# jhardenberg/smmregrid

Measured on NVIDIA B200. Metric: regridded source points/sec, 0.1deg->1deg remapcon, higher is better.
Workload: dtype f64

## Files before the change

### include/smmregrid_b200.h

```cpp
#ifndef SMMREGRID_B200_H
#define SMMREGRID_B200_H

#include <stdint.h>

#ifdef __cplusplus
extern "C" {
#endif

#define SMM_OK 0
#define SMM_ERR_INVALID 1
#define SMM_ERR_RANGE 2
#define SMM_ERR_CUDA 3
#define SMM_ERR_ALLOC 4
#define SMM_ERR_DTYPE 5

#define SMM_F32 0
#define SMM_F64 1
#define SMM_I16 2

#define SMM_KERNEL_STAGED 1
#define SMM_KERNEL_GATHER 2
#define SMM_KERNEL_COMPACT 3

#define SMM_SUM_AUTO 0
// ... 100 lines not shown

typedef struct smm_host_plan smm_host_plan;
int smm_host_plan_build(int64_t n_src, int64_t n_dst, int64_t nnz,
                        const int32_t *src_address, const int32_t *dst_address,
                        const double *remap_matrix, int32_t num_wgts, int32_t index_base,
                        const smm_create_opts *opts, smm_host_plan **out);
int smm_host_plan_info(const smm_host_plan *p, smm_info *out, int64_t *n_segs_out);
int smm_host_plan_copy(const smm_host_plan *p, int32_t *rowptr, int32_t *col, double *val,
                       int32_t *tiles, uint32_t *segs, double *wplan, uint16_t *iplan);
int smm_host_plan_rowmap(const smm_host_plan *p, int32_t *rowmap);
int smm_host_plan_gather_rows(const smm_host_plan *p, int32_t *rows);
int smm_host_plan_rowslot(const smm_host_plan *p, int32_t *rowslot);
int smm_host_plan_compact(const smm_host_plan *p, int64_t *n_touched_out, int64_t *n_blocks_out,
                          int32_t *tcols, int32_t *blk_ptr, int32_t *rcol);
void smm_host_plan_free(smm_host_plan *p);

int smm_copy_ceiling(int32_t device, void *host, int64_t bytes, int32_t direction, int32_t reps,
                     double *seconds_out);

int64_t smm_launch_count(void);

const char *smm_last_error(void);
const char *smm_version(void);

#ifdef __cplusplus
}
#endif
#endif
```

### smmregrid_b200/_lib.py

```python
from __future__ import annotations

import ctypes
import os

from . import _build

SMM_OK, SMM_ERR_INVALID, SMM_ERR_RANGE, SMM_ERR_CUDA, SMM_ERR_ALLOC, SMM_ERR_DTYPE = range(6)
SMM_F32, SMM_F64, SMM_I16 = 0, 1, 2
SMM_KERNEL_STAGED, SMM_KERNEL_GATHER, SMM_KERNEL_COMPACT = 1, 2, 3
KERNEL_NAMES = {SMM_KERNEL_STAGED: "staged", SMM_KERNEL_GATHER: "gather"}
KERNEL_CODES = {None: 0, "auto": 0, "staged": SMM_KERNEL_STAGED, "gather": SMM_KERNEL_GATHER,
                "compact": SMM_KERNEL_COMPACT}
SMM_SUM_AUTO, SMM_SUM_FAST, SMM_SUM_REFERENCE = 0, 1, 2
SUMMATION_CODES = {None: SMM_SUM_AUTO, "auto": SMM_SUM_AUTO, "fast": SMM_SUM_FAST, "reference": SMM_SUM_REFERENCE}
SUMMATION_NAMES = {SMM_SUM_FAST: "fast", SMM_SUM_REFERENCE: "reference"}

i32, i64, f64 = ctypes.c_int32, ctypes.c_int64, ctypes.c_double
vp = ctypes.c_void_p
P = ctypes.POINTER


class SmmInfo(ctypes.Structure):
    _fields_ = [
        ("n_src", i64), ("n_dst", i64), ("nnz", i64),
# ... 50 lines not shown
    "smm_set_dst_mask": (ctypes.c_int, [vp, i32, vp, vp]),
    "smm_apply": (ctypes.c_int, [vp, i32, vp, i32, i64, i64, vp, i32, i64, i32, f64, P(SmmApplyOpts), vp]),
    "smm_apply_levels": (ctypes.c_int, [vp, i32, vp, vp, i32, i64, i64, i64, vp, i32, i64, i64, vp, f64,
                                        P(SmmApplyOpts), vp]),
    "smm_apply_host": (ctypes.c_int, [vp, i32, vp, i32, i64, i64, vp, i32, i64, i32, f64, P(SmmApplyOpts), i64]),
    "smm_apply_levels_host": (ctypes.c_int, [vp, i32, vp, vp, i32, i64, vp, i32, vp, f64, P(SmmApplyOpts), i64]),
    "smm_nan_variation": (ctypes.c_int, [vp, i32, i64, i64, i64, P(i64), vp]),
    "smm_host_plan_build": (ctypes.c_int, [i64, i64, i64, vp, vp, vp, i32, i32, P(SmmCreateOpts), P(vp)]),
    "smm_host_plan_info": (ctypes.c_int, [vp, P(SmmInfo), P(i64)]),
    "smm_host_plan_copy": (ctypes.c_int, [vp, vp, vp, vp, vp, vp, vp, vp]),
    "smm_host_plan_rowmap": (ctypes.c_int, [vp, vp]),
    "smm_host_plan_rowslot": (ctypes.c_int, [vp, vp]),
    "smm_host_plan_gather_rows": (ctypes.c_int, [vp, vp]),
    "smm_host_plan_compact": (ctypes.c_int, [vp, P(i64), P(i64), vp, vp, vp]),
    "smm_host_plan_free": (None, [vp]),
    "smm_copy_ceiling": (ctypes.c_int, [i32, vp, i64, i32, i32, P(f64)]),
    "smm_launch_count": (i64, []),
    "smm_last_error": (ctypes.c_char_p, []),
    "smm_version": (ctypes.c_char_p, []),
}

_lib = None


class SmmError(RuntimeError):
    pass


def lib_path() -> str:
    return os.environ.get("SMM_LIB_PATH") or _build.LIB_PATH
# ... 28 lines not shown
```

### smmregrid_b200/csrc/smm_api.cu

```cuda
#include <cuda_runtime.h>

#include <algorithm>
#include <atomic>
#include <chrono>
#include <cmath>
#include <cstdio>
#include <cstdlib>
#include <cstring>
#include <mutex>
#include <string>
#include <thread>
#include <vector>

#include <sched.h>
#if defined(__x86_64__) || defined(_M_X64)
#include <emmintrin.h>
#endif

#include "../../include/smmregrid_b200.h"
#include "smm_internal.h"
#include "smm_aux_kernels.cuh"
#include "smm_plan.h"

using namespace smm;
// ... 331 lines not shown
    return e ? std::atoi(e) : dflt;
}

#define SMM_DTYPE_DISPATCH(FN, ...)                                                                           \
    ((x_dtype == SMM_I16)                                                                                     \
         ? ((opt.dec_dtype == SMM_F32)                                                                        \
                ? (y_dtype == SMM_F32 ? FN<I16F32, float>(__VA_ARGS__) : FN<I16F32, double>(__VA_ARGS__))     \
                : (y_dtype == SMM_F32 ? FN<I16F64, float>(__VA_ARGS__) : FN<I16F64, double>(__VA_ARGS__)))    \
     : (x_dtype == SMM_F32 && y_dtype == SMM_F32) ? FN<float, float>(__VA_ARGS__)                             \
     : (x_dtype == SMM_F32 && y_dtype == SMM_F64) ? FN<float, double>(__VA_ARGS__)                            \
     : (x_dtype == SMM_F64 && y_dtype == SMM_F32) ? FN<double, float>(__VA_ARGS__)                            \
                                                  : FN<double, double>(__VA_ARGS__))

size_t x_elem_bytes(int32_t x_dtype) { return x_dtype == SMM_I16 ? 2 : x_dtype == SMM_F32 ? 4 : 8; }

int64_t pick_chunks(int64_t B, int64_t blocks_total, int64_t slots, double bytes_per_row, double prologue_us,
                    int64_t multiple, int64_t &chunk)
{
    static const int k_min_rows = std::max(1, env_int("SMM_MIN_ROWS_PER_ITEM", 8));
    static const int k_waves = env_int("SMM_WAVES", 0);
    const double t_us = static_cast<double>(B) * bytes_per_row / 6.5e6;
    double waves = k_waves > 0 ? k_waves : std::sqrt(t_us / (2.0 * prologue_us));
    waves = std::min(32.0, std::max(1.0, waves));
    const double items = waves * static_cast<double>(slots);
    int64_t nchunks = static_cast<int64_t>(items / static_cast<double>(std::max<int64_t>(blocks_total, 1)) + 0.5);
    const int64_t max_chunks = std::max<int64_t>(1, B / k_min_rows);
    nchunks = std::max<int64_t>(1, std::min<int64_t>({nchunks, max_chunks, 65535}));
    chunk = (B + nchunks - 1) / nchunks;
    chunk = (chunk + multiple - 1) / multiple * multiple;
    return (B + chunk - 1) / chunk;
}

constexpr int kCompactUnavailable = -1;

struct ApplyOpts {
    int kernel = 0;
    double renorm_min_valid = -1.0;
// ... 103 lines not shown
        if (!ok && opt.kernel == SMM_KERNEL_STAGED)
            return fail(SMM_ERR_INVALID, "staged kernel forced but unavailable for level " +
                                             std::to_string(s.level) + ": " +
                                             (L.staged ? std::string("slab alignment / footprint size")
                                                       : L.why_not_staged));
        (ok ? staged : gather).push_back(s);
        if (ok && L.n_gather_rows > 0) gather_lists.push_back(s);
    }

    ApplyArgs a{};
    a.B = B; a.x_bstride = xbs; a.y_bstride = ybs; a.remap_area_min = area_min;
    a.renorm_min_valid = opt.renorm_min_valid;
    a.dec = opt.dec;
    static const uint32_t k_debug_flags = static_cast<uint32_t>(env_int("SMM_DEBUG_STREAM_ONLY", 0)) & 3u;
    static const int k_max_stages = std::max(2, env_int("SMM_MAX_STAGES", kMaxStages));
    a.debug_flags = k_debug_flags;

    auto fill_job = [&](const JobSpec &s, LevelJob &j) {
        const LevelDev &L = h->levels[s.level];
        j.tiles = L.tiles; j.segs = L.segs; j.wplan = L.wplan; j.iplan = L.iplan; j.rowmap = L.rowmap;
        j.rowptr = L.rowptr; j.col = L.col; j.val = L.val;
        j.imask = L.imask; j.frac = L.frac;
        j.x = s.x; j.y = s.y; j.masked = s.masked; j.nrows = 0;
    };

    const size_t staged_groups = (staged.size() + kMaxJobs - 1) / kMaxJobs;
    const size_t staged_per = staged_groups ? (staged.size() + staged_groups - 1) / staged_groups : 1;
    for (size_t g0 = 0; g0 < staged.size();) {
        size_t g1 = g0;
        JobBatch jb{};
// ... 24 lines not shown
        {
            const size_t budget = (nct == 256 ? half : h->smem_optin) - std::min(stage_off, half);
            nb_rows = static_cast<int>(std::min<size_t>(nb_rows, std::max<size_t>(1, budget / (4 * row_bytes))));
        }
        nb_rows = static_cast<int>(std::max<int64_t>(1, std::min<int64_t>({nb_rows, 8, B})));
        if (ordl) {
            nb_rows = (B >= 2 && stage_off + 4 * row_bytes <= h->smem_optin) ? 2 : 1;
            while (nb_rows >= 2 && nb_rows + 2 <= 8 && nb_rows + 2 <= B &&
                   stage_off + 3 * static_cast<size_t>(nb_rows + 2) * row_bytes <= h->smem_optin)
                nb_rows += 2;
        }
        const size_t stage_bytes = row_bytes * nb_rows;
        int64_t chunk = 0;
        const double row_bytes_hbm = static_cast<double>(g1 - g0) *
                                     (static_cast<double>(a.n_src) * sx + static_cast<double>(a.n_dst) * (y_dtype == SMM_F32 ? 4 : 8));
        const int ctas_per_sm = (!ordl && nct == 256) ? 2 : 1;
        const int64_t nchunks = pick_chunks(B, tiles_total, static_cast<int64_t>(h->sm_count) * ctas_per_sm,
                                            row_bytes_hbm, ordl ? 6.0 : (nct == 256 ? 2.5 : 4.0), nb_rows, chunk);
        a.chunk = chunk; a.nchunks = static_cast<int32_t>(nchunks);
        size_t S = (!ordl && nct == 256 && half > stage_off) ? (half - stage_off) / stage_bytes : 0;
        if (S < 3) S = (h->smem_optin - stage_off) / stage_bytes;
        S = std::min<size_t>(S, kMaxStages);
        S = std::min<size_t>(S, static_cast<size_t>(k_max_stages));
        if (S < 2) return fail(SMM_ERR_INVALID, "internal: staged footprint does not fit");
        a.nstages = static_cast<int32_t>(S);
        a.stage_bytes = static_cast<uint32_t>(stage_bytes);
        a.row_bytes = static_cast<uint32_t>(row_bytes);
        a.rows_per_stage = nb_rows;
        a.stage_off = static_cast<uint32_t>(stage_off);
        const size_t smem = stage_off + S * stage_bytes;
        int64_t max_tiles = 0;
        jb.njobs = static_cast<int32_t>(g1 - g0);
        for (size_t g = g0; g < g1; ++g) {
            LevelJob &j = jb.jobs[g - g0];
            fill_job(staged[g], j);
            j.nblocks = h->levels[staged[g].level].ntiles;
            j.item0 = 0;
            max_tiles = std::max<int64_t>(max_tiles, j.nblocks);
        }
        g0 = g1;
        if (max_tiles == 0) continue;
        const dim3 grid(static_cast<unsigned>(max_tiles), static_cast<unsigned>(nchunks), static_cast<unsigned>(jb.njobs));
        static const int k_ord_tpr = env_int("SMM_ORD_TPR", 0);
        const int tpr = (ordl && nb_rows >= 2 && (k_ord_tpr == 2 || (k_ord_tpr == 0 && nct <= 128))) ? 2 : 1;
        const int rc = ordl ? SMM_DTYPE_DISPATCH(launch_ordered_t, h->device, nct, tpr, grid, smem, st, jb, a)
                            : SMM_DTYPE_DISPATCH(launch_staged_t, h->device, lpr, kpl, nct, packed, ord, grid, smem, st, jb, a);
        if (rc) return rc;
    }

    {
        std::vector<JobSpec> plain;
        for (const JobSpec &sp : gather) {
            const LevelDev &L = h->levels[sp.level];
            const double gather_cost = static_cast<double>(L.nnz) * 120.0;
            const double compact_cost = 1.2 * (static_cast<double>(L.n_src) + static_cast<double>(L.touched) +
                                               static_cast<double>(L.nnz)) * static_cast<double>(sx);
            bool use = L.rcol && opt.renorm_min_valid < 0.0 && opt.kernel != SMM_KERNEL_GATHER;
// ... 582 lines not shown
    smm_host_plan *p = new (std::nothrow) smm_host_plan();
    if (!p) return fail(SMM_ERR_ALLOC, "host allocation failed");
    std::vector<HostCsr> csrs;
    std::vector<HostPlan> plans;
    bool ref_order = false;
    const int64_t ll = nnz;
    const int rc = build_host_operator(1, &ll, nnz, n_src, n_dst, src_address, dst_address, remap_matrix, num_wgts,
                                       index_base, opts, 148, csrs, plans, ref_order, p->cache_hit);
    if (rc) { delete p; return rc; }
    p->csr = std::move(csrs[0]);
    p->plan = std::move(plans[0]);
    *out = p;
    return SMM_OK;
}

int smm_host_plan_info(const smm_host_plan *p, smm_info *out, int64_t *n_segs_out)
{
    if (!p || !out) return fail(SMM_ERR_INVALID, "null argument");
    std::memset(out, 0, sizeof(*out));
    out->n_src = p->csr.n_src; out->n_dst = p->csr.n_dst;
    out->nnz = static_cast<int64_t>(p->csr.col.size());
    out->n_levels = 1;
    out->kernel = p->plan.ok ? SMM_KERNEL_STAGED : SMM_KERNEL_GATHER;
    out->lanes_per_row = p->plan.lpr; out->links_per_lane = p->plan.kpl;
    out->rows_per_tile = p->plan.rows_per_tile;
    out->n_tiles = p->plan.ok ? static_cast<int32_t>(p->plan.tiles.size()) : 0;
    out->max_row_nnz = p->csr.max_row_nnz;
    out->max_tile_segments = p->plan.max_tile_segments;
    out->consumer_threads = p->plan.nct;
    out->rows_reordered = (p->plan.ok && p->plan.reordered) ? 1 : 0;
// ... 107 lines not shown
```

### smmregrid_b200/csrc/smm_common.h

```cpp
#pragma once
#include <cstdint>

namespace smm {

constexpr int kMaxConsumerThreads = 512;
constexpr int kMaxStages = 12;
constexpr int kSegAlign = 8;
constexpr int kSegGap = 32;
constexpr int kSmemHeader = 256;
constexpr int kMaxJobs = 128;
constexpr int kGatherThreads = 256;
constexpr int kGatherBT = 4;

#ifndef SMM_COMPACT_BC
#define SMM_COMPACT_BC 64
#endif
#ifndef SMM_COMPACT_W
#define SMM_COMPACT_W 256
#endif
constexpr int kCompactBC = SMM_COMPACT_BC;
constexpr int kCompactW = SMM_COMPACT_W;

struct Seg {
    uint32_t src;
// ... 32 lines not shown

struct JobBatch {
    LevelJob jobs[kMaxJobs];
    int32_t njobs;
    int32_t pad;
};

struct Decode {
    double scale, offset;
    float scale_f, offset_f;
    int32_t fill[4];
    uint32_t sign_xor;
    float bias_f;
};

struct ApplyArgs {
    int64_t B;
    int64_t x_bstride;
    int64_t y_bstride;
    int64_t n_src, n_dst;
    int64_t chunk;
    int32_t nchunks;
    int32_t nstages;
    uint32_t stage_bytes;
    uint32_t row_bytes;
    int32_t rows_per_stage;
    uint32_t stage_off;
    double remap_area_min;
    double renorm_min_valid;
    uint32_t debug_flags;
    int32_t ord_k;
    uint32_t wimg_off, oimg_off;
    Decode dec;
};

}
```

### smmregrid_b200/csrc/smm_kernels.cuh

```cuda
#pragma once
#include <cuda_runtime.h>
#include <math_constants.h>
#include <cuda/std/type_traits>

#include "smm_common.h"

namespace smm {


__device__ __forceinline__ uint32_t smem_u32(const void *p)
{
    return static_cast<uint32_t>(__cvta_generic_to_shared(p));
}
__device__ __forceinline__ void mbar_init(uint32_t bar, uint32_t count)
{
    asm volatile("mbarrier.init.shared::cta.b64 [%0], %1;" ::"r"(bar), "r"(count) : "memory");
}
__device__ __forceinline__ void mbar_fence_init()
{
    asm volatile("fence.mbarrier_init.release.cluster;" ::: "memory");
}
__device__ __forceinline__ void mbar_arrive(uint32_t bar)
{
    asm volatile("mbarrier.arrive.shared::cta.b64 _, [%0];" ::"r"(bar) : "memory");
// ... 166 lines not shown
#endif
}

__device__ __forceinline__ const LevelJob &find_job(const JobBatch &jb, int item, int &j)
{
    int lo = 0, hi = jb.njobs - 1;
#pragma unroll 1
    while (lo < hi) {
        const int mid = (lo + hi + 1) >> 1;
        if (item >= jb.jobs[mid].item0) lo = mid; else hi = mid - 1;
    }
    j = lo;
    return jb.jobs[j];
}


template <typename TX> __device__ __forceinline__ TX lds(uint32_t addr);
template <> __device__ __forceinline__ float lds<float>(uint32_t addr)
{
    float v;
    asm volatile("ld.shared.f32 %0, [%1];" : "=f"(v) : "r"(addr));
    return v;
}
template <> __device__ __forceinline__ double lds<double>(uint32_t addr)
{
    double v;
    asm volatile("ld.shared.f64 %0, [%1];" : "=d"(v) : "r"(addr));
    return v;
}
template <> __device__ __forceinline__ uint16_t lds<uint16_t>(uint32_t addr)
// ... 158 lines not shown
#ifndef SMM_PRODUCERS_512
#define SMM_PRODUCERS_512 4
#endif
__host__ __device__ constexpr int producer_warps(int nct) { return nct == 512 ? SMM_PRODUCERS_512 : 4; }
constexpr int kProducerRegs = 40;
#ifndef SMM_CONSUMER_REGS_512
#define SMM_CONSUMER_REGS_512 104
#endif
__host__ __device__ constexpr int consumer_regs(int nct) { return nct == 512 ? SMM_CONSUMER_REGS_512 : 96; }

struct SegB { uint32_t dst, len; uint64_t src; };

template <typename TX>
__device__ __forceinline__ void produce_stages(const LevelJob &job, const ApplyArgs &a, const TileDesc &td,
                                               const SegB *ssegs, uint32_t full_addr, uint32_t empty_addr,
                                               uint32_t stages_addr, int p, int nwarps, int lane, int64_t b0, int64_t b1)
{
    const int per_stage = td.nseg * a.rows_per_stage;
    const int active = per_stage >= 3 * nwarps ? nwarps : (per_stage + 2) / 3 > 0 ? (per_stage + 2) / 3 : 1;
    if (p >= active) return;
    const uint64_t policy = l2_evict_first_policy();
    const char *xbase = static_cast<const char *>(job.x);
    const uint32_t tile_bytes = static_cast<uint32_t>(td.elems) * sizeof(xs_t<TX>);
    const int NB = a.rows_per_stage;
    const int S = a.nstages;
    const int64_t xrow_stride = a.x_bstride * static_cast<int64_t>(sizeof(xs_t<TX>));
    int s = 0;
    uint32_t ph = 0;
    for (int64_t g = b0; g < b1; g += NB) {
        const int nb = (g + NB <= b1) ? NB : static_cast<int>(b1 - g);
        mbar_wait(empty_addr + 8 * s, ph ^ 1u);
        const uint32_t fb = full_addr + 8 * s;
        if (p == 0 && lane == 0) mbar_arrive_expect_tx(fb, tile_bytes * static_cast<uint32_t>(nb));
        const char *xg = xbase + g * xrow_stride;
        const uint32_t sbase = stages_addr + static_cast<uint32_t>(s) * a.stage_bytes;
        const int ncopies = nb * td.nseg;
        for (int i = p + active * lane; i < ncopies; i += 32 * active) {
            const int n = i / td.nseg;
            const SegB e = ssegs[i - n * td.nseg];
            tma_bulk_g2s(sbase + static_cast<uint32_t>(n) * a.row_bytes + e.dst, xg + n * xrow_stride + e.src, e.len,
                         fb, policy);
        }
        if (++s == S) { s = 0; ph ^= 1u; }
    }
}

template <typename TX, typename TY, int LPR, int KPL, int NCT, bool PACKED = false, bool ORD = false>
__global__ void __launch_bounds__(NCT + 32 * producer_warps(NCT), NCT == 256 ? 2 : 1)
staged_kernel(const __grid_constant__ JobBatch jb, const __grid_constant__ ApplyArgs a)
{
    constexpr int kProducerWarps = producer_warps(NCT);
    constexpr int kThreads = NCT + 32 * kProducerWarps;
    constexpr int kConsumerWarps = NCT / 32;
    extern __shared__ __align__(128) unsigned char smem[];
    const int tid = threadIdx.x;
    const int warp = tid >> 5;
    const int lane = tid & 31;

    const LevelJob &job = jb.jobs[blockIdx.z];
    const int tile = blockIdx.x;
    const int chunk = blockIdx.y;
    if (tile >= job.nblocks) return;
    const int64_t b0 = static_cast<int64_t>(chunk) * a.chunk;
    const int64_t b1 = (b0 + a.chunk < a.B) ? b0 + a.chunk : a.B;
    const TileDesc td = job.tiles[tile];

    SegB *ssegs = reinterpret_cast<SegB *>(smem + kSmemHeader);
    const uint32_t smem_addr = pin_reg(smem_u32(smem));
    const uint32_t full_addr = smem_addr, empty_addr = smem_addr + 8 * kMaxStages;
    const uint32_t stages_addr = smem_u32(smem) + a.stage_off;
    const int S = a.nstages;

    for (int i = tid; i < td.nseg; i += kThreads) {
        const Seg sg = job.segs[td.seg0 + i];
        ssegs[i] = SegB{sg.dst * static_cast<uint32_t>(sizeof(xs_t<TX>)), sg.len * static_cast<uint32_t>(sizeof(xs_t<TX>)),
                        static_cast<uint64_t>(sg.src) * sizeof(xs_t<TX>)};
    }
    if (tid == 0) {
        for (int s = 0; s < S; ++s) {
            mbar_init(full_addr + 8 * s, 1);
            mbar_init(empty_addr + 8 * s, kConsumerWarps);
        }
        mbar_fence_init();
    }
    __syncthreads();

    if (warp >= kConsumerWarps) {
        asm volatile("setmaxnreg.dec.sync.aligned.u32 %0;" ::"n"(kProducerRegs));
        produce_stages<TX>(job, a, td, ssegs, full_addr, empty_addr, stages_addr, warp - kConsumerWarps, kProducerWarps,
                           lane, b0, b1);
    } else {
        asm volatile("setmaxnreg.inc.sync.aligned.u32 %0;" ::"n"(consumer_regs(NCT)));
        const int r_in = tid / LPR;
        const int l_in = tid % LPR;
        const bool valid = r_in < td.nrows;
        const int row = (!PACKED && job.rowmap && valid) ? job.rowmap[td.row0 + r_in] : td.row0 + r_in;

        double w[KPL];
        uint32_t off[KPL];
        {
            const size_t base = static_cast<size_t>(tile) * KPL * NCT + tid;
#pragma unroll
            for (int k = 0; k < KPL; ++k) {
                w[k] = __ldg(job.wplan + base + static_cast<size_t>(k) * NCT);
                off[k] = stages_addr + static_cast<uint32_t>(__ldg(job.iplan + base + static_cast<size_t>(k) * NCT)) *
                                           static_cast<uint32_t>(sizeof(xs_t<TX>));
            }
        }
        if constexpr (PACKED) {
            static_assert(LPR == 1 && KPL == 16, "packed rows: 4 sub-rows of 4 links per thread");
            int rs[4];
            uint32_t flags = 0;
#pragma unroll
            for (int u = 0; u < 4; ++u) {
                rs[u] = __ldg(job.rowmap + (static_cast<size_t>(tile) * 4 + u) * NCT + tid);
                if (rs[u] == -2) flags |= 1u << u;
                if (rs[u] >= 0) {
                    bool dead = false;
                    if (job.masked && job.imask[rs[u]] == 0) dead = true;
                    if (a.remap_area_min > 0.0 && job.frac[rs[u]] < a.remap_area_min) dead = true;
                    if (dead) flags |= 16u << u;
                }
            }
            uint32_t dm[4];
#pragma unroll
            for (int u = 0; u < 4; ++u) {
                dm[u] = (flags & (16u << u)) ? 0x7ff80000u : 0u;
                asm volatile("" : "+r"(dm[u]));
            }
            TY *yb = static_cast<TY *>(job.y) + b0 * a.y_bstride;
            const xs_t<TX> *xp = static_cast<const xs_t<TX> *>(job.x) + b0 * a.x_bstride;
            const bool stream_only = (a.debug_flags & 1u) != 0;
            const int NB = a.rows_per_stage;
            bool prefer_fill = false;
            uint32_t n_done = 0;
            int s = 0;
            uint32_t ph = 0;
            for (int64_t g = b0; g < b1; g += NB) {
                const int nb = (g + NB <= b1) ? NB : static_cast<int>(b1 - g);
                mbar_wait(full_addr + 8 * s, ph);
                uint32_t sb = static_cast<uint32_t>(s) * a.stage_bytes;
#pragma unroll 1
                for (int n = 0; n < nb; ++n, sb += a.row_bytes, yb += a.y_bstride, xp += a.x_bstride) {
                    double s4[4] = {0.0, 0.0, 0.0, 0.0};
                    if (!stream_only) {
                        const bool probe = !prefer_fill || (n_done & 15u) == 0;
                        ++n_done;
                        if (probe) {
                            if constexpr (ORD) lane_chain4<TX, false>(sb, off, w, flags, s4, a.dec);
                            else lane_sum4<TX, false>(sb, off, w, s4, a.dec);
                            prefer_fill = __any_sync(0xffffffffu, not_finite((s4[0] + s4[1]) + (s4[2] + s4[3])));
                        }
                        if (prefer_fill) {
                            if constexpr (ORD) lane_chain4<TX, true>(sb, off, w, flags, s4, a.dec);
                            else lane_sum4<TX, true>(sb, off, w, s4, a.dec);
                        }
                    }
                    if (n == nb - 1) {
                        __syncwarp();
                        if (lane == 0) mbar_arrive(empty_addr + 8 * s);
                    }
                    double acc[4];
                    acc[3] = s4[3];
                    if constexpr (ORD) {
                        acc[2] = (flags & 8u) ? acc[3] : s4[2];
                        acc[1] = (flags & 4u) ? acc[2] : s4[1];
                        acc[0] = (flags & 2u) ? acc[1] : s4[0];
                    } else {
                        acc[2] = s4[2] + ((flags & 8u) ? acc[3] : 0.0);
                        acc[1] = s4[1] + ((flags & 4u) ? acc[2] : 0.0);
                        acc[0] = s4[0] + ((flags & 2u) ? acc[1] : 0.0);
                    }
                    const int hi_max = max(max(__double2hiint(acc[0]), __double2hiint(acc[1])),
                                           max(__double2hiint(acc[2]), __double2hiint(acc[3])));
                    if (__any_sync(0xffffffffu, hi_max >= 0x43E12C7B)) {
#pragma unroll
                        for (int u = 0; u < 4; ++u) {
                            if (rs[u] >= 0)
                                store_y(yb + rs[u], finish<TY, ORD>(acc[u], (flags & (16u << u)) != 0,
                                                                    [&]() { return replay<TX>(job.rowptr, job.col, job.val, rs[u], xp, a.dec); }));
                        }
                    } else {
#pragma unroll
                        for (int u = 0; u < 4; ++u) {
                            if (rs[u] >= 0)
                                store_y(yb + rs[u], static_cast<TY>(__hiloint2double(__double2hiint(acc[u]) | static_cast<int>(dm[u]),
                                                                                     __double2loint(acc[u]))));
                        }
                    }
                }
                if (++s == S) { s = 0; ph ^= 1u; }
            }
            return;
        }
        bool dead = false;
        if (valid) {
            if (job.masked && job.imask[row] == 0) dead = true;
            if (a.remap_area_min > 0.0 && job.frac[row] < a.remap_area_min) dead = true;
        }
        TY *yp = static_cast<TY *>(job.y) + row + b0 * a.y_bstride;
        const xs_t<TX> *xp = static_cast<const xs_t<TX> *>(job.x) + b0 * a.x_bstride;
        const bool stream_only = (a.debug_flags & 1u) != 0;

        const int NB = a.rows_per_stage;
        bool prefer_fill = false;
        uint32_t n_done = 0;
        int s = 0;
        uint32_t ph = 0;
        for (int64_t g = b0; g < b1; g += NB) {
            const int nb = (g + NB <= b1) ? NB : static_cast<int>(b1 - g);
            mbar_wait(full_addr + 8 * s, ph);
            uint32_t sb = static_cast<uint32_t>(s) * a.stage_bytes;
#pragma unroll 1
            for (int n = 0; n < nb; ++n, sb += a.row_bytes, yp += a.y_bstride, xp += a.x_bstride) {
                double acc = 0.0;
                bool renormed = false;
                if (!stream_only) {
                    const bool probe = !prefer_fill || (n_done & 15u) == 0;
                    ++n_done;
                    auto row_sum = [&](auto fill) -> double {
                        if constexpr (ORD) return lane_sum_ordered<TX, LPR, KPL, decltype(fill)::value>(sb, off, w, l_in, a.dec);
                        else return lane_sum<TX, KPL, decltype(fill)::value>(sb, off, w, a.dec);
                    };
                    if (!probe) {
                        acc = row_sum(cuda::std::true_type{});
                    } else {
                        prefer_fill = false;
                        acc = row_sum(cuda::std::false_type{});
                        if (__any_sync(0xffffffffu, not_finite(acc))) {
                            if (a.renorm_min_valid < 0.0) {
                                acc = row_sum(cuda::std::true_type{});
                                prefer_fill = true;
                            } else {
                                double s3[3];
                                const size_t base = static_cast<size_t>(tile) * KPL * NCT + tid;
                                if constexpr (XElem<TX>::kPacked)
                                    lane_sum_valid<TX, KPL, NCT>(job.wplan, job.iplan, base, stages_addr + sb, s3, a.dec);
                                else
                                    lane_sum_valid<TX, KPL, NCT>(job.wplan, job.iplan, base, stages_addr + sb, s3);
                                acc = renormalise(group_sum<LPR>(s3[0]), group_sum<LPR>(s3[1]), group_sum<LPR>(s3[2]),
                                                  a.renorm_min_valid);
                                renormed = true;
                            }
                        }
                    }
                }
                if (n == nb - 1) {
                    __syncwarp();
                    if (lane == 0) mbar_arrive(empty_addr + 8 * s);
                }
                if (renormed) {
                    if (l_in == 0 && valid) store_y(yp, static_cast<TY>(dead ? CUDART_NAN : acc));
                } else {
                    if constexpr (!ORD) acc = group_sum<LPR>(acc);
                    if (l_in == 0 && valid && !(a.debug_flags & 2u)) {
                        if (a.renorm_min_valid < 0.0)
                            store_y(yp, finish<TY, ORD>(acc, dead, [&]() { return replay<TX>(job.rowptr, job.col, job.val, row, xp, a.dec); }));
                        else
                            store_y(yp, static_cast<TY>(dead ? CUDART_NAN : acc));
                    }
                }
            }
            if (++s == S) { s = 0; ph ^= 1u; }
        }
    }
}


__device__ __forceinline__ double lds_f64(uint32_t addr)
{
    double v;
    asm volatile("ld.shared.f64 %0, [%1];" : "=d"(v) : "r"(addr));
    return v;
}
__device__ __forceinline__ uint32_t lds_u32(uint32_t addr)
{
    uint32_t v;
    asm volatile("ld.shared.u32 %0, [%1];" : "=r"(v) : "r"(addr));
// ... 130 lines not shown
        for (int i = tid; i < K * R; i += kThreads) {
            wimg[i] = __ldg(job.wplan + ibase + i);
            oimg[i] = stages_addr + static_cast<uint32_t>(__ldg(job.iplan + ibase + i)) * static_cast<uint32_t>(sizeof(xs_t<TX>));
        }
    }
    if (tid == 0) {
        for (int s = 0; s < S; ++s) {
            mbar_init(full_addr + 8 * s, 1);
            mbar_init(empty_addr + 8 * s, kConsumerWarps);
        }
        mbar_fence_init();
    }
    __syncthreads();

    if (warp >= kConsumerWarps) {
        produce_stages<TX>(job, a, td, ssegs, full_addr, empty_addr, stages_addr, warp - kConsumerWarps,
                           kOrderedProducerWarps, lane, b0, b1);
        return;
    }
    if constexpr (TPR == 2) {
        if (tid < R)
            ordered_consume_half<TX, TY, R, 0>(job, a, td, smem_u32(wimg), smem_u32(oimg), full_addr, empty_addr, tid,
                                               lane, b0, b1);
        else
            ordered_consume_half<TX, TY, R, 1>(job, a, td, smem_u32(wimg), smem_u32(oimg), full_addr, empty_addr,
                                               tid - R, lane, b0, b1);
        return;
    }
    asm volatile("barrier.sync.aligned 1, %0;" ::"n"(R) : "memory");
    const bool valid = tid < td.nrows;
    const int row = (job.rowmap && valid) ? job.rowmap[td.row0 + tid] : td.row0 + tid;
    bool dead = false;
// ... 337 lines not shown
```

Before: 1655 billion.

## Make staged kernel persistent with a work-split cursor across tiles and batch bands

```diff
diff --git a/include/smmregrid_b200.h b/include/smmregrid_b200.h
--- a/include/smmregrid_b200.h
+++ b/include/smmregrid_b200.h
@@ -138,6 +138,8 @@
 int smm_host_plan_compact(const smm_host_plan *p, int64_t *n_touched_out, int64_t *n_blocks_out,
                           int32_t *tcols, int32_t *blk_ptr, int32_t *rcol);
 void smm_host_plan_free(smm_host_plan *p);
+int smm_staged_split(int64_t n_tiles, int64_t B, int64_t rows_per_item, int32_t ctas, int32_t cta,
+                     int64_t *items, int64_t cap, int64_t *n_items);
 
 int smm_copy_ceiling(int32_t device, void *host, int64_t bytes, int32_t direction, int32_t reps,
                      double *seconds_out);
diff --git a/smmregrid_b200/_lib.py b/smmregrid_b200/_lib.py
--- a/smmregrid_b200/_lib.py
+++ b/smmregrid_b200/_lib.py
@@ -88,6 +88,7 @@
     "smm_host_plan_gather_rows": (ctypes.c_int, [vp, vp]),
     "smm_host_plan_compact": (ctypes.c_int, [vp, P(i64), P(i64), vp, vp, vp]),
     "smm_host_plan_free": (None, [vp]),
+    "smm_staged_split": (ctypes.c_int, [i64, i64, i64, i32, i32, vp, i64, P(i64)]),
     "smm_copy_ceiling": (ctypes.c_int, [i32, vp, i64, i32, i32, P(f64)]),
     "smm_launch_count": (i64, []),
     "smm_last_error": (ctypes.c_char_p, []),
diff --git a/smmregrid_b200/csrc/smm_api.cu b/smmregrid_b200/csrc/smm_api.cu
--- a/smmregrid_b200/csrc/smm_api.cu
+++ b/smmregrid_b200/csrc/smm_api.cu
@@ -369,13 +369,14 @@
 
 size_t x_elem_bytes(int32_t x_dtype) { return x_dtype == SMM_I16 ? 2 : x_dtype == SMM_F32 ? 4 : 8; }
 
+constexpr double kPersistentWaves = 8.0;
 int64_t pick_chunks(int64_t B, int64_t blocks_total, int64_t slots, double bytes_per_row, double prologue_us,
                     int64_t multiple, int64_t &chunk)
 {
     static const int k_min_rows = std::max(1, env_int("SMM_MIN_ROWS_PER_ITEM", 8));
     static const int k_waves = env_int("SMM_WAVES", 0);
     const double t_us = static_cast<double>(B) * bytes_per_row / 6.5e6;
-    double waves = k_waves > 0 ? k_waves : std::sqrt(t_us / (2.0 * prologue_us));
+    double waves = k_waves > 0 ? k_waves : prologue_us > 0.0 ? std::sqrt(t_us / (2.0 * prologue_us)) : kPersistentWaves;
     waves = std::min(32.0, std::max(1.0, waves));
     const double items = waves * static_cast<double>(slots);
     int64_t nchunks = static_cast<int64_t>(items / static_cast<double>(std::max<int64_t>(blocks_total, 1)) + 0.5);
@@ -509,6 +510,7 @@
     a.dec = opt.dec;
     static const uint32_t k_debug_flags = static_cast<uint32_t>(env_int("SMM_DEBUG_STREAM_ONLY", 0)) & 3u;
     static const int k_max_stages = std::max(2, env_int("SMM_MAX_STAGES", kMaxStages));
+    static const bool k_persistent = env_int("SMM_PERSISTENT", 1) != 0;
     a.debug_flags = k_debug_flags;
 
     auto fill_job = [&](const JobSpec &s, LevelJob &j) {
@@ -563,33 +565,41 @@
         int64_t chunk = 0;
         const double row_bytes_hbm = static_cast<double>(g1 - g0) *
                                      (static_cast<double>(a.n_src) * sx + static_cast<double>(a.n_dst) * (y_dtype == SMM_F32 ? 4 : 8));
+        size_t S = (!ordl && nct == 256 && half > stage_off) ? (half - stage_off) / stage_bytes : 0;
+        const bool persist = k_persistent && S >= 3;
         const int ctas_per_sm = (!ordl && nct == 256) ? 2 : 1;
-        const int64_t nchunks = pick_chunks(B, tiles_total, static_cast<int64_t>(h->sm_count) * ctas_per_sm,
-                                            row_bytes_hbm, ordl ? 6.0 : (nct == 256 ? 2.5 : 4.0), nb_rows, chunk);
-        a.chunk = chunk; a.nchunks = static_cast<int32_t>(nchunks);
-        size_t S = (!ordl && nct == 256 && half > stage_off) ? (half - stage_off) / stage_bytes : 0;
         if (S < 3) S = (h->smem_optin - stage_off) / stage_bytes;
         S = std::min<size_t>(S, kMaxStages);
         S = std::min<size_t>(S, static_cast<size_t>(k_max_stages));
         if (S < 2) return fail(SMM_ERR_INVALID, "internal: staged footprint does not fit");
+        const int64_t slots = static_cast<int64_t>(h->sm_count) * ctas_per_sm;
+        const int64_t nchunks = pick_chunks(B, tiles_total, slots, row_bytes_hbm,
+                                            persist ? 0.0 : ordl ? 6.0 : (nct == 256 ? 2.5 : 4.0), nb_rows, chunk);
+        a.chunk = chunk; a.nchunks = static_cast<int32_t>(nchunks);
         a.nstages = static_cast<int32_t>(S);
         a.stage_bytes = static_cast<uint32_t>(stage_bytes);
         a.row_bytes = static_cast<uint32_t>(row_bytes);
         a.rows_per_stage = nb_rows;
         a.stage_off = static_cast<uint32_t>(stage_off);
         const size_t smem = stage_off + S * stage_bytes;
-        int64_t max_tiles = 0;
+        int64_t max_tiles = 0, tile0 = 0;
         jb.njobs = static_cast<int32_t>(g1 - g0);
         for (size_t g = g0; g < g1; ++g) {
             LevelJob &j = jb.jobs[g - g0];
             fill_job(staged[g], j);
             j.nblocks = h->levels[staged[g].level].ntiles;
-            j.item0 = 0;
+            j.item0 = static_cast<int32_t>(tile0);
+            tile0 += j.nblocks;
             max_tiles = std::max<int64_t>(max_tiles, j.nblocks);
         }
         g0 = g1;
         if (max_tiles == 0) continue;
-        const dim3 grid(static_cast<unsigned>(max_tiles), static_cast<unsigned>(nchunks), static_cast<unsigned>(jb.njobs));
+        a.split = Split{};
+        dim3 grid(static_cast<unsigned>(max_tiles), static_cast<unsigned>(nchunks), static_cast<unsigned>(jb.njobs));
+        if (persist) {
+            a.split = make_split(tiles_total, B, std::min(chunk, B), std::min<int64_t>(slots, tiles_total * B));
+            grid = dim3(static_cast<unsigned>(a.split.G));
+        }
         static const int k_ord_tpr = env_int("SMM_ORD_TPR", 0);
         const int tpr = (ordl && nb_rows >= 2 && (k_ord_tpr == 2 || (k_ord_tpr == 0 && nct <= 128))) ? 2 : 1;
         const int rc = ordl ? SMM_DTYPE_DISPATCH(launch_ordered_t, h->device, nct, tpr, grid, smem, st, jb, a)
@@ -1202,6 +1212,22 @@
     return SMM_OK;
 }
 
+int smm_staged_split(int64_t n_tiles, int64_t B, int64_t rows_per_item, int32_t ctas, int32_t cta,
+                     int64_t *items, int64_t cap, int64_t *n_items)
+{
+    if (n_tiles < 1 || B < 1 || rows_per_item < 1 || ctas < 1 || cta < 0 || cta >= ctas || cap < 0 || !n_items ||
+        (cap > 0 && !items))
+        return fail(SMM_ERR_INVALID, "smm_staged_split: invalid argument");
+    const Split s = make_split(n_tiles, B, rows_per_item, ctas);
+    SplitCursor cur(s, cta);
+    int64_t n = 0, t, b0, b1;
+    for (; cur.next(s, cta, t, b0, b1); ++n) {
+        if (n < cap) { items[3 * n] = t; items[3 * n + 1] = b0; items[3 * n + 2] = b1; }
+    }
+    *n_items = n;
+    return SMM_OK;
+}
+
 int smm_host_plan_info(const smm_host_plan *p, smm_info *out, int64_t *n_segs_out)
 {
     if (!p || !out) return fail(SMM_ERR_INVALID, "null argument");
diff --git a/smmregrid_b200/csrc/smm_common.h b/smmregrid_b200/csrc/smm_common.h
--- a/smmregrid_b200/csrc/smm_common.h
+++ b/smmregrid_b200/csrc/smm_common.h
@@ -7,7 +7,8 @@
 constexpr int kMaxStages = 12;
 constexpr int kSegAlign = 8;
 constexpr int kSegGap = 32;
-constexpr int kSmemHeader = 256;
+constexpr int kSmemHeader = 512;
+constexpr int kStageDescOff = 192, kCursorOff = 384, kWorkItemOff = 416;
 constexpr int kMaxJobs = 128;
 constexpr int kGatherThreads = 256;
 constexpr int kGatherBT = 4;
@@ -70,6 +71,82 @@
     float bias_f;
 };
 
+#ifdef __CUDACC__
+#define SMM_HD __host__ __device__ __forceinline__
+#else
+#define SMM_HD inline
+#endif
+
+struct Split {
+    int64_t T;
+    int64_t B;
+    int64_t rows;
+    int64_t bands;
+    int64_t rounds;
+    int64_t rest_items;
+    int64_t tail;
+    int64_t G;
+};
+
+SMM_HD Split make_split(int64_t T, int64_t B, int64_t rows, int64_t G)
+{
+    Split s{};
+    s.T = T; s.B = B; s.rows = rows; s.G = G;
+    s.bands = B / rows;
+    s.rounds = T * s.bands / G;
+    s.rest_items = T * s.bands - s.rounds * G;
+    s.tail = s.rest_items * rows + T * (B - s.bands * rows);
+    return s;
+}
+
+struct SplitCursor {
+    int64_t k, u, u1;
+
+    SMM_HD SplitCursor(const Split &s, int64_t c) : k(0), u(s.G ? c * s.tail / s.G : 0), u1(s.G ? (c + 1) * s.tail / s.G : 0) {}
+
+    SMM_HD bool next(const Split &s, int64_t c, int64_t &t, int64_t &b0, int64_t &b1)
+    {
+        if (k < s.rounds) {
+            const int64_t i = k++ * s.G + c, band = i / s.T;
+            t = i - band * s.T;
+            b0 = band * s.rows;
+            b1 = b0 + s.rows;
+            return true;
+        }
+        if (u >= u1) return false;
+        const int64_t head = s.rest_items * s.rows;
+        int64_t len;
+        if (u < head) {
+            const int64_t q = u / s.rows, i = s.rounds * s.G + q, band = i / s.T;
+            t = i - band * s.T;
+            b0 = band * s.rows + (u - q * s.rows);
+            len = ((q + 1) * s.rows < u1 ? (q + 1) * s.rows : u1) - u;
+        } else {
+            const int64_t rr = s.B - s.bands * s.rows, w = u - head;
+            t = w / rr;
+            const int64_t off = w - t * rr;
+            b0 = s.bands * s.rows + off;
+            len = (rr - off < u1 - u) ? rr - off : u1 - u;
+        }
+        b1 = b0 + len;
+        u += len;
+        return true;
+    }
+};
+
+struct WorkItem {
+    int32_t j, tile;
+    int64_t b0, b1;
+};
+
+struct alignas(16) StageDesc {
+    int64_t b0;
+    int32_t tile;
+    int16_t j;
+    uint8_t nb;
+    bool first;
+};
+
 struct ApplyArgs {
     int64_t B;
     int64_t x_bstride;
@@ -88,6 +165,7 @@
     int32_t ord_k;
     uint32_t wimg_off, oimg_off;
     Decode dec;
+    Split split;
 };
 
 }
diff --git a/smmregrid_b200/csrc/smm_kernels.cuh b/smmregrid_b200/csrc/smm_kernels.cuh
--- a/smmregrid_b200/csrc/smm_kernels.cuh
+++ b/smmregrid_b200/csrc/smm_kernels.cuh
@@ -204,6 +204,25 @@
     return jb.jobs[j];
 }
 
+__device__ __forceinline__ WorkItem next_item(const JobBatch &jb, const ApplyArgs &a, SplitCursor &cur)
+{
+    WorkItem it{-1, 0, 0, 0};
+    if (a.split.T > 0) {
+        int64_t t;
+        if (cur.next(a.split, blockIdx.x, t, it.b0, it.b1)) {
+            int j;
+            it.tile = static_cast<int>(t) - find_job(jb, static_cast<int>(t), j).item0;
+            it.j = j;
+        }
+    } else if (cur.k++ == 0 && static_cast<int>(blockIdx.x) < jb.jobs[blockIdx.z].nblocks) {
+        it.j = blockIdx.z;
+        it.tile = blockIdx.x;
+        it.b0 = static_cast<int64_t>(blockIdx.y) * a.chunk;
+        it.b1 = (it.b0 + a.chunk < a.B) ? it.b0 + a.chunk : a.B;
+    }
+    return it;
+}
+
 
 template <typename TX> __device__ __forceinline__ TX lds(uint32_t addr);
 template <> __device__ __forceinline__ float lds<float>(uint32_t addr)
@@ -392,24 +411,32 @@
 template <typename TX>
 __device__ __forceinline__ void produce_stages(const LevelJob &job, const ApplyArgs &a, const TileDesc &td,
                                                const SegB *ssegs, uint32_t full_addr, uint32_t empty_addr,
-                                               uint32_t stages_addr, int p, int nwarps, int lane, int64_t b0, int64_t b1)
-{
-    const int per_stage = td.nseg * a.rows_per_stage;
+                                               uint32_t stages_addr, int p, int nwarps, int lane, const WorkItem &it,
+                                               StageDesc *sdesc, int &s, uint32_t &ph)
+{
+    const int64_t b0 = it.b0, b1 = it.b1;
+    const int NB = a.rows_per_stage;
+    const int S = a.nstages;
+    const int per_stage = td.nseg * NB;
     const int active = per_stage >= 3 * nwarps ? nwarps : (per_stage + 2) / 3 > 0 ? (per_stage + 2) / 3 : 1;
-    if (p >= active) return;
+    if (p >= active) {
+        const int t = s + static_cast<int>((b1 - b0 + NB - 1) / NB);
+        ph ^= static_cast<uint32_t>(t / S) & 1u;
+        s = t % S;
+        return;
+    }
     const uint64_t policy = l2_evict_first_policy();
     const char *xbase = static_cast<const char *>(job.x);
     const uint32_t tile_bytes = static_cast<uint32_t>(td.elems) * sizeof(xs_t<TX>);
-    const int NB = a.rows_per_stage;
-    const int S = a.nstages;
     const int64_t xrow_stride = a.x_bstride * static_cast<int64_t>(sizeof(xs_t<TX>));
-    int s = 0;
-    uint32_t ph = 0;
     for (int64_t g = b0; g < b1; g += NB) {
         const int nb = (g + NB <= b1) ? NB : static_cast<int>(b1 - g);
         mbar_wait(empty_addr + 8 * s, ph ^ 1u);
         const uint32_t fb = full_addr + 8 * s;
-        if (p == 0 && lane == 0) mbar_arrive_expect_tx(fb, tile_bytes * static_cast<uint32_t>(nb));
+        if (p == 0 && lane == 0) {
+            if (sdesc) sdesc[s] = StageDesc{g, it.tile, static_cast<int16_t>(it.j), static_cast<uint8_t>(nb), g == b0};
+            mbar_arrive_expect_tx(fb, tile_bytes * static_cast<uint32_t>(nb));
+        }
         const char *xg = xbase + g * xrow_stride;
         const uint32_t sbase = stages_addr + static_cast<uint32_t>(s) * a.stage_bytes;
         const int ncopies = nb * td.nseg;
@@ -428,32 +455,17 @@
 staged_kernel(const __grid_constant__ JobBatch jb, const __grid_constant__ ApplyArgs a)
 {
     constexpr int kProducerWarps = producer_warps(NCT);
-    constexpr int kThreads = NCT + 32 * kProducerWarps;
     constexpr int kConsumerWarps = NCT / 32;
     extern __shared__ __align__(128) unsigned char smem[];
     const int tid = threadIdx.x;
     const int warp = tid >> 5;
     const int lane = tid & 31;
 
-    const LevelJob &job = jb.jobs[blockIdx.z];
-    const int tile = blockIdx.x;
-    const int chunk = blockIdx.y;
-    if (tile >= job.nblocks) return;
-    const int64_t b0 = static_cast<int64_t>(chunk) * a.chunk;
-    const int64_t b1 = (b0 + a.chunk < a.B) ? b0 + a.chunk : a.B;
-    const TileDesc td = job.tiles[tile];
-
-    SegB *ssegs = reinterpret_cast<SegB *>(smem + kSmemHeader);
     const uint32_t smem_addr = pin_reg(smem_u32(smem));
     const uint32_t full_addr = smem_addr, empty_addr = smem_addr + 8 * kMaxStages;
     const uint32_t stages_addr = smem_u32(smem) + a.stage_off;
     const int S = a.nstages;
 
-    for (int i = tid; i < td.nseg; i += kThreads) {
-        const Seg sg = job.segs[td.seg0 + i];
-        ssegs[i] = SegB{sg.dst * static_cast<uint32_t>(sizeof(xs_t<TX>)), sg.len * static_cast<uint32_t>(sizeof(xs_t<TX>)),
-                        static_cast<uint64_t>(sg.src) * sizeof(xs_t<TX>)};
-    }
     if (tid == 0) {
         for (int s = 0; s < S; ++s) {
             mbar_init(full_addr + 8 * s, 1);
@@ -463,183 +475,217 @@
     }
     __syncthreads();
 
+    StageDesc *sdesc = reinterpret_cast<StageDesc *>(smem + kStageDescOff);
     if (warp >= kConsumerWarps) {
         asm volatile("setmaxnreg.dec.sync.aligned.u32 %0;" ::"n"(kProducerRegs));
-        produce_stages<TX>(job, a, td, ssegs, full_addr, empty_addr, stages_addr, warp - kConsumerWarps, kProducerWarps,
-                           lane, b0, b1);
+        const int p = warp - kConsumerWarps;
+        const bool leader = p == 0 && lane == 0;
+        WorkItem *item = reinterpret_cast<WorkItem *>(smem + kWorkItemOff);
+        SplitCursor *cur = reinterpret_cast<SplitCursor *>(smem + kCursorOff);
+        if (leader) *cur = SplitCursor(a.split, blockIdx.x);
+        SegB *ssegs = reinterpret_cast<SegB *>(smem + kSmemHeader);
+        int s = 0;
+        uint32_t ph = 0;
+        for (;;) {
+            if (leader) *item = next_item(jb, a, *cur);
+            asm volatile("barrier.sync.aligned 1, %0;" ::"n"(32 * kProducerWarps) : "memory");
+            const WorkItem it = *item;
+            if (it.j < 0) break;
+            const LevelJob &job = jb.jobs[it.j];
+            const TileDesc td = job.tiles[it.tile];
+            for (int i = tid - NCT; i < td.nseg; i += 32 * kProducerWarps) {
+                const Seg sg = job.segs[td.seg0 + i];
+                ssegs[i] = SegB{sg.dst * static_cast<uint32_t>(sizeof(xs_t<TX>)), sg.len * static_cast<uint32_t>(sizeof(xs_t<TX>)),
+                                static_cast<uint64_t>(sg.src) * sizeof(xs_t<TX>)};
+            }
+            asm volatile("barrier.sync.aligned 1, %0;" ::"n"(32 * kProducerWarps) : "memory");
+            produce_stages<TX>(job, a, td, ssegs, full_addr, empty_addr, stages_addr, p, kProducerWarps, lane, it, sdesc,
+                               s, ph);
+        }
+        if (leader) {
+            mbar_wait(empty_addr + 8 * s, ph ^ 1u);
+            sdesc[s] = StageDesc{0, 0, 0, 0, true};
+            mbar_arrive(full_addr + 8 * s);
+        }
     } else {
         asm volatile("setmaxnreg.inc.sync.aligned.u32 %0;" ::"n"(consumer_regs(NCT)));
         const int r_in = tid / LPR;
         const int l_in = tid % LPR;
-        const bool valid = r_in < td.nrows;
-        const int row = (!PACKED && job.rowmap && valid) ? job.rowmap[td.row0 + r_in] : td.row0 + r_in;
-
-        double w[KPL];
-        uint32_t off[KPL];
-        {
-            const size_t base = static_cast<size_t>(tile) * KPL * NCT + tid;
-#pragma unroll
-            for (int k = 0; k < KPL; ++k) {
-                w[k] = __ldg(job.wplan + base + static_cast<size_t>(k) * NCT);
-                off[k] = stages_addr + static_cast<uint32_t>(__ldg(job.iplan + base + static_cast<size_t>(k) * NCT)) *
-                                           static_cast<uint32_t>(sizeof(xs_t<TX>));
-            }
-        }
-        if constexpr (PACKED) {
-            static_assert(LPR == 1 && KPL == 16, "packed rows: 4 sub-rows of 4 links per thread");
-            int rs[4];
-            uint32_t flags = 0;
-#pragma unroll
-            for (int u = 0; u < 4; ++u) {
-                rs[u] = __ldg(job.rowmap + (static_cast<size_t>(tile) * 4 + u) * NCT + tid);
-                if (rs[u] == -2) flags |= 1u << u;
-                if (rs[u] >= 0) {
-                    bool dead = false;
-                    if (job.masked && job.imask[rs[u]] == 0) dead = true;
-                    if (a.remap_area_min > 0.0 && job.frac[rs[u]] < a.remap_area_min) dead = true;
-                    if (dead) flags |= 16u << u;
+        const bool stream_only = (a.debug_flags & 1u) != 0;
+        bool prefer_fill = false;
+        uint32_t n_done = 0;
+        int s = 0;
+        uint32_t ph = 0;
+        mbar_wait(full_addr, 0);
+        for (;;) {
+            const StageDesc d = sdesc[s];
+            if (d.nb == 0) break;
+            const int tile = d.tile;
+            const LevelJob &job = jb.jobs[d.j];
+            const TileDesc td = job.tiles[tile];
+            const bool valid = r_in < td.nrows;
+            const int row = (!PACKED && job.rowmap && valid) ? job.rowmap[td.row0 + r_in] : td.row0 + r_in;
+
+            double w[KPL];
+            uint32_t off[KPL];
+            {
+                const size_t base = static_cast<size_t>(tile) * KPL * NCT + tid;
+#pragma unroll
+                for (int k = 0; k < KPL; ++k) {
+                    w[k] = __ldg(job.wplan + base + static_cast<size_t>(k) * NCT);
+                    off[k] = stages_addr + static_cast<uint32_t>(__ldg(job.iplan + base + static_cast<size_t>(k) * NCT)) *
+                                               static_cast<uint32_t>(sizeof(xs_t<TX>));
                 }
             }
-            uint32_t dm[4];
-#pragma unroll
-            for (int u = 0; u < 4; ++u) {
-                dm[u] = (flags & (16u << u)) ? 0x7ff80000u : 0u;
-                asm volatile("" : "+r"(dm[u]));
-            }
-            TY *yb = static_cast<TY *>(job.y) + b0 * a.y_bstride;
-            const xs_t<TX> *xp = static_cast<const xs_t<TX> *>(job.x) + b0 * a.x_bstride;
-            const bool stream_only = (a.debug_flags & 1u) != 0;
-            const int NB = a.rows_per_stage;
-            bool prefer_fill = false;
-            uint32_t n_done = 0;
-            int s = 0;
-            uint32_t ph = 0;
-            for (int64_t g = b0; g < b1; g += NB) {
-                const int nb = (g + NB <= b1) ? NB : static_cast<int>(b1 - g);
-                mbar_wait(full_addr + 8 * s, ph);
+            if constexpr (PACKED) {
+                static_assert(LPR == 1 && KPL == 16, "packed rows: 4 sub-rows of 4 links per thread");
+                int rs[4];
+                uint32_t flags = 0;
+#pragma unroll
+                for (int u = 0; u < 4; ++u) {
+                    rs[u] = __ldg(job.rowmap + (static_cast<size_t>(tile) * 4 + u) * NCT + tid);
+                    if (rs[u] == -2) flags |= 1u << u;
+                    if (rs[u] >= 0) {
+                        bool dead = false;
+                        if (job.masked && job.imask[rs[u]] == 0) dead = true;
+                        if (a.remap_area_min > 0.0 && job.frac[rs[u]] < a.remap_area_min) dead = true;
+                        if (dead) flags |= 16u << u;
+                    }
+                }
+                uint32_t dm[4];
+#pragma unroll
+                for (int u = 0; u < 4; ++u) {
+                    dm[u] = (flags & (16u << u)) ? 0x7ff80000u : 0u;
+                    asm volatile("" : "+r"(dm[u]));
+                }
+                const int64_t b0 = d.b0;
+                int bi = 0;
+                for (int nb = d.nb;;) {
+                    uint32_t sb = static_cast<uint32_t>(s) * a.stage_bytes;
+#pragma unroll 1
+                    for (int n = 0; n < nb; ++n, sb += a.row_bytes, ++bi) {
+                        TY *yb = static_cast<TY *>(job.y) + (b0 + bi) * a.y_bstride;
+                        double s4[4] = {0.0, 0.0, 0.0, 0.0};
+                        if (!stream_only) {
+                            const bool probe = !prefer_fill || (n_done & 15u) == 0;
+                            ++n_done;
+                            if (probe) {
+                                if constexpr (ORD) lane_chain4<TX, false>(sb, off, w, flags, s4, a.dec);
+                                else lane_sum4<TX, false>(sb, off, w, s4, a.dec);
+                                prefer_fill = __any_sync(0xffffffffu, not_finite((s4[0] + s4[1]) + (s4[2] + s4[3])));
+                            }
+                            if (prefer_fill) {
+                                if constexpr (ORD) lane_chain4<TX, true>(sb, off, w, flags, s4, a.dec);
+                                else lane_sum4<TX, true>(sb, off, w, s4, a.dec);
+                            }
+                        }
+                        if (n == nb - 1) {
+                            __syncwarp();
+                            if (lane == 0) mbar_arrive(empty_addr + 8 * s);
+                        }
+                        double acc[4];
+                        acc[3] = s4[3];
+                        if constexpr (ORD) {
+                            acc[2] = (flags & 8u) ? acc[3] : s4[2];
+                            acc[1] = (flags & 4u) ? acc[2] : s4[1];
+                            acc[0] = (flags & 2u) ? acc[1] : s4[0];
+                        } else {
+                            acc[2] = s4[2] + ((flags & 8u) ? acc[3] : 0.0);
+                            acc[1] = s4[1] + ((flags & 4u) ? acc[2] : 0.0);
+                            acc[0] = s4[0] + ((flags & 2u) ? acc[1] : 0.0);
+                        }
+                        const int hi_max = max(max(__double2hiint(acc[0]), __double2hiint(acc[1])),
+                                               max(__double2hiint(acc[2]), __double2hiint(acc[3])));
+                        if (__any_sync(0xffffffffu, hi_max >= 0x43E12C7B)) {
+#pragma unroll
+                            for (int u = 0; u < 4; ++u) {
+                                if (rs[u] >= 0)
+                                    store_y(yb + rs[u], finish<TY, ORD>(acc[u], (flags & (16u << u)) != 0,
+                                                                        [&]() {
+                                        const xs_t<TX> *xp = static_cast<const xs_t<TX> *>(job.x) + (b0 + bi) * a.x_bstride;
+                                        return replay<TX>(job.rowptr, job.col, job.val, rs[u], xp, a.dec);
+                                    }));
+                            }
+                        } else {
+#pragma unroll
+                            for (int u = 0; u < 4; ++u) {
+                                if (rs[u] >= 0)
+                                    store_y(yb + rs[u], static_cast<TY>(__hiloint2double(__double2hiint(acc[u]) | static_cast<int>(dm[u]),
+                                                                                         __double2loint(acc[u]))));
+                            }
+                        }
+                    }
+                    if (++s == S) { s = 0; ph ^= 1u; }
+                    mbar_wait(full_addr + 8 * s, ph);
+                    if (sdesc[s].first) break;
+                    nb = sdesc[s].nb;
+                }
+                continue;
+            }
+            bool dead = false;
+            if (valid) {
+                if (job.masked && job.imask[row] == 0) dead = true;
+                if (a.remap_area_min > 0.0 && job.frac[row] < a.remap_area_min) dead = true;
+            }
+            TY *yp = static_cast<TY *>(job.y) + row + d.b0 * a.y_bstride;
+            const xs_t<TX> *xp = static_cast<const xs_t<TX> *>(job.x) + d.b0 * a.x_bstride;
+            for (int nb = d.nb;;) {
                 uint32_t sb = static_cast<uint32_t>(s) * a.stage_bytes;
 #pragma unroll 1
-                for (int n = 0; n < nb; ++n, sb += a.row_bytes, yb += a.y_bstride, xp += a.x_bstride) {
-                    double s4[4] = {0.0, 0.0, 0.0, 0.0};
+                for (int n = 0; n < nb; ++n, sb += a.row_bytes, yp += a.y_bstride, xp += a.x_bstride) {
+                    double acc = 0.0;
+                    bool renormed = false;
                     if (!stream_only) {
                         const bool probe = !prefer_fill || (n_done & 15u) == 0;
                         ++n_done;
-                        if (probe) {
-                            if constexpr (ORD) lane_chain4<TX, false>(sb, off, w, flags, s4, a.dec);
-                            else lane_sum4<TX, false>(sb, off, w, s4, a.dec);
-                            prefer_fill = __any_sync(0xffffffffu, not_finite((s4[0] + s4[1]) + (s4[2] + s4[3])));
-                        }
-                        if (prefer_fill) {
-                            if constexpr (ORD) lane_chain4<TX, true>(sb, off, w, flags, s4, a.dec);
-                            else lane_sum4<TX, true>(sb, off, w, s4, a.dec);
+                        auto row_sum = [&](auto fill) -> double {
+                            if constexpr (ORD) return lane_sum_ordered<TX, LPR, KPL, decltype(fill)::value>(sb, off, w, l_in, a.dec);
+                            else return lane_sum<TX, KPL, decltype(fill)::value>(sb, off, w, a.dec);
+                        };
+                        if (!probe) {
+                            acc = row_sum(cuda::std::true_type{});
+                        } else {
+                            prefer_fill = false;
+                            acc = row_sum(cuda::std::false_type{});
+                            if (__any_sync(0xffffffffu, not_finite(acc))) {
+                                if (a.renorm_min_valid < 0.0) {
+                                    acc = row_sum(cuda::std::true_type{});
+                                    prefer_fill = true;
+                                } else {
+                                    double s3[3];
+                                    const size_t base = static_cast<size_t>(tile) * KPL * NCT + tid;
+                                    if constexpr (XElem<TX>::kPacked)
+                                        lane_sum_valid<TX, KPL, NCT>(job.wplan, job.iplan, base, stages_addr + sb, s3, a.dec);
+                                    else
+                                        lane_sum_valid<TX, KPL, NCT>(job.wplan, job.iplan, base, stages_addr + sb, s3);
+                                    acc = renormalise(group_sum<LPR>(s3[0]), group_sum<LPR>(s3[1]), group_sum<LPR>(s3[2]),
+                                                      a.renorm_min_valid);
+                                    renormed = true;
+                                }
+                            }
                         }
                     }
                     if (n == nb - 1) {
                         __syncwarp();
                         if (lane == 0) mbar_arrive(empty_addr + 8 * s);
                     }
-                    double acc[4];
-                    acc[3] = s4[3];
-                    if constexpr (ORD) {
-                        acc[2] = (flags & 8u) ? acc[3] : s4[2];
-                        acc[1] = (flags & 4u) ? acc[2] : s4[1];
-                        acc[0] = (flags & 2u) ? acc[1] : s4[0];
+                    if (renormed) {
+                        if (l_in == 0 && valid) store_y(yp, static_cast<TY>(dead ? CUDART_NAN : acc));
                     } else {
-                        acc[2] = s4[2] + ((flags & 8u) ? acc[3] : 0.0);
-                        acc[1] = s4[1] + ((flags & 4u) ? acc[2] : 0.0);
-                        acc[0] = s4[0] + ((flags & 2u) ? acc[1] : 0.0);
-                    }
-                    const int hi_max = max(max(__double2hiint(acc[0]), __double2hiint(acc[1])),
-                                           max(__double2hiint(acc[2]), __double2hiint(acc[3])));
-                    if (__any_sync(0xffffffffu, hi_max >= 0x43E12C7B)) {
-#pragma unroll
-                        for (int u = 0; u < 4; ++u) {
-                            if (rs[u] >= 0)
-                                store_y(yb + rs[u], finish<TY, ORD>(acc[u], (flags & (16u << u)) != 0,
-                                                                    [&]() { return replay<TX>(job.rowptr, job.col, job.val, rs[u], xp, a.dec); }));
-                        }
-                    } else {
-#pragma unroll
-                        for (int u = 0; u < 4; ++u) {
-                            if (rs[u] >= 0)
-                                store_y(yb + rs[u], static_cast<TY>(__hiloint2double(__double2hiint(acc[u]) | static_cast<int>(dm[u]),
-                                                                                     __double2loint(acc[u]))));
+                        if constexpr (!ORD) acc = group_sum<LPR>(acc);
+                        if (l_in == 0 && valid && !(a.debug_flags & 2u)) {
+                            if (a.renorm_min_valid < 0.0)
+                                store_y(yp, finish<TY, ORD>(acc, dead, [&]() { return replay<TX>(job.rowptr, job.col, job.val, row, xp, a.dec); }));
+                            else
+                                store_y(yp, static_cast<TY>(dead ? CUDART_NAN : acc));
                         }
                     }
                 }
                 if (++s == S) { s = 0; ph ^= 1u; }
-            }
-            return;
-        }
-        bool dead = false;
-        if (valid) {
-            if (job.masked && job.imask[row] == 0) dead = true;
-            if (a.remap_area_min > 0.0 && job.frac[row] < a.remap_area_min) dead = true;
-        }
-        TY *yp = static_cast<TY *>(job.y) + row + b0 * a.y_bstride;
-        const xs_t<TX> *xp = static_cast<const xs_t<TX> *>(job.x) + b0 * a.x_bstride;
-        const bool stream_only = (a.debug_flags & 1u) != 0;
-
-        const int NB = a.rows_per_stage;
-        bool prefer_fill = false;
-        uint32_t n_done = 0;
-        int s = 0;
-        uint32_t ph = 0;
-        for (int64_t g = b0; g < b1; g += NB) {
-            const int nb = (g + NB <= b1) ? NB : static_cast<int>(b1 - g);
-            mbar_wait(full_addr + 8 * s, ph);
-            uint32_t sb = static_cast<uint32_t>(s) * a.stage_bytes;
-#pragma unroll 1
-            for (int n = 0; n < nb; ++n, sb += a.row_bytes, yp += a.y_bstride, xp += a.x_bstride) {
-                double acc = 0.0;
-                bool renormed = false;
-                if (!stream_only) {
-                    const bool probe = !prefer_fill || (n_done & 15u) == 0;
-                    ++n_done;
-                    auto row_sum = [&](auto fill) -> double {
-                        if constexpr (ORD) return lane_sum_ordered<TX, LPR, KPL, decltype(fill)::value>(sb, off, w, l_in, a.dec);
-                        else return lane_sum<TX, KPL, decltype(fill)::value>(sb, off, w, a.dec);
-                    };
-                    if (!probe) {
-                        acc = row_sum(cuda::std::true_type{});
-                    } else {
-                        prefer_fill = false;
-                        acc = row_sum(cuda::std::false_type{});
-                        if (__any_sync(0xffffffffu, not_finite(acc))) {
-                            if (a.renorm_min_valid < 0.0) {
-                                acc = row_sum(cuda::std::true_type{});
-                                prefer_fill = true;
-                            } else {
-                                double s3[3];
-                                const size_t base = static_cast<size_t>(tile) * KPL * NCT + tid;
-                                if constexpr (XElem<TX>::kPacked)
-                                    lane_sum_valid<TX, KPL, NCT>(job.wplan, job.iplan, base, stages_addr + sb, s3, a.dec);
-                                else
-                                    lane_sum_valid<TX, KPL, NCT>(job.wplan, job.iplan, base, stages_addr + sb, s3);
-                                acc = renormalise(group_sum<LPR>(s3[0]), group_sum<LPR>(s3[1]), group_sum<LPR>(s3[2]),
-                                                  a.renorm_min_valid);
-                                renormed = true;
-                            }
-                        }
-                    }
-                }
-                if (n == nb - 1) {
-                    __syncwarp();
-                    if (lane == 0) mbar_arrive(empty_addr + 8 * s);
-                }
-                if (renormed) {
-                    if (l_in == 0 && valid) store_y(yp, static_cast<TY>(dead ? CUDART_NAN : acc));
-                } else {
-                    if constexpr (!ORD) acc = group_sum<LPR>(acc);
-                    if (l_in == 0 && valid && !(a.debug_flags & 2u)) {
-                        if (a.renorm_min_valid < 0.0)
-                            store_y(yp, finish<TY, ORD>(acc, dead, [&]() { return replay<TX>(job.rowptr, job.col, job.val, row, xp, a.dec); }));
-                        else
-                            store_y(yp, static_cast<TY>(dead ? CUDART_NAN : acc));
-                    }
-                }
-            }
-            if (++s == S) { s = 0; ph ^= 1u; }
+                mbar_wait(full_addr + 8 * s, ph);
+                if (sdesc[s].first) break;
+                nb = sdesc[s].nb;
+            }
         }
     }
 }
@@ -800,8 +846,10 @@
     __syncthreads();
 
     if (warp >= kConsumerWarps) {
+        int s = 0;
+        uint32_t ph = 0;
         produce_stages<TX>(job, a, td, ssegs, full_addr, empty_addr, stages_addr, warp - kConsumerWarps,
-                           kOrderedProducerWarps, lane, b0, b1);
+                           kOrderedProducerWarps, lane, WorkItem{0, 0, b0, b1}, nullptr, s, ph);
         return;
     }
     if constexpr (TPR == 2) {
```

After: 1646 billion (median of 6 runs). About the same (-0.6%).
